# Duy1230/Map-Reduced-Approach-for-Vietnamese-Long-Document-Summarization

Hardware: AMD Instinct MI355X
Metric: map-phase chunks/sec (2k-tok chunk, 256-tok summary) at 1/2/4/8 MI355X (higher is better)
Workload: dtype f16

## Files before the change

### include/mapsum.h

```cpp
#ifndef MAPSUM_H
#define MAPSUM_H

#include <stddef.h>
#include <stdint.h>

#ifdef __cplusplus
extern "C" {
#endif

#define MS_ABI_VERSION 3

#define MS_OK 0
#define MS_EIO -5
#define MS_ENOMEM -12
#define MS_EBUSY -16
#define MS_EINVAL -22
#define MS_ENOSPC -28

#define MS_FINISH_EOS 1
#define MS_FINISH_LENGTH 2
#define MS_FINISH_ERROR 3

#define MS_FLAG_IGNORE_EOS 1u

// ... 71 lines not shown
int ms_quant_manifest(const ms_engine* e, int32_t* triples, int32_t cap);
int ms_declare_weight_q(ms_engine* e, int32_t tensor, int32_t layer, int32_t ggml_type);

int ms_submit(ms_engine* e, const int32_t* ids, int32_t n, int32_t num_predict,
              uint32_t flags, uint64_t tag);
int ms_set_eos_ids(ms_engine* e, const int32_t* ids, int32_t n);
int ms_step(ms_engine* e);
int ms_poll(ms_engine* e, ms_result* out, int32_t cap);
int ms_pending(const ms_engine* e);
int ms_get_stats(const ms_engine* e, ms_stats* out);
int ms_reset_stats(ms_engine* e);
int ms_set_profiling(ms_engine* e, uint32_t class_mask);
int ms_trace_push(const char* name);
int ms_trace_pop(void);
int ms_synchronize(ms_engine* e);
int ms_set_persist(ms_engine* e, int32_t on);
#define MS_DBG_KPOOL 0
#define MS_DBG_VPOOL 1
#define MS_DBG_DECODE_LOGITS 2
#define MS_DBG_DECODE_X 3
int ms_debug_read(ms_engine* e, int32_t which, int64_t offset, void* host, int64_t bytes);
int ms_debug_pk_stamps(uint64_t* out, int32_t n);
int ms_debug_a2_stamps(uint64_t* out, int32_t n);

int ms_forward(ms_engine* e, const int32_t* ids, int32_t n, int32_t n_layers_run,
               float* hidden_out, float* logits_out);
int ms_forward_packed(ms_engine* e, const int32_t* ids, const int32_t* lens, int32_t n_seqs,
                      int32_t n_layers_run, float* hidden_out, float* logits_out);
int ms_submit_forced(ms_engine* e, const int32_t* ids, int32_t n, const int32_t* forced,
                     int32_t n_forced, int32_t num_predict, uint32_t flags, uint64_t tag);

#define MS_EPI_STORE_F16 0
#define MS_EPI_ADD_F32 1
#define MS_EPI_SWIGLU 2
#define MS_EPI_STORE_F32 3
#define MS_EPI_ARGMAX 5
int ms_op_gemm(const void* A, const void* W, void* out, int32_t M, int32_t N, int32_t K,
               int32_t ldo, int32_t epilogue, void* stream);
int ms_op_gemm_resid(const void* A, const void* W, float* x, void* xg_out, const void* gamma, float* ssq_out,
                     int32_t M, int32_t N, int32_t K, void* stream);
int ms_gemm_resid_tiles(int32_t M, int32_t N);
int ms_set_gemm_variant(int32_t variant);
int ms_set_qgemv_gs(int32_t on);
int ms_set_attn_tuning(int32_t combine_grp, int32_t order);
int ms_set_dgemm_kh(int32_t kh);
int ms_set_dgemm_wn(int32_t wn);
// ... 35 lines not shown
```

### map-reduced-approach-for-vietnamese-long-document-summarization_amd/csrc/engine.cpp

```cpp
#include <hip/hip_runtime.h>

#include <algorithm>
#include <cmath>
#include <cstdio>
#include <cstdlib>
#include <cstring>
#include <deque>
#include <array>
#include <functional>
#include <map>
#include <tuple>
#include <memory>
#include <stdexcept>
#include <string>
#include <vector>

#if MS_HAVE_ROCTX
#include <rocprofiler-sdk-roctx/roctx.h>
#else
static inline int roctxRangePushA(const char*) { return 0; }
static inline int roctxRangePop() { return 0; }
#endif

#include "kernels.h"
// ... 128 lines not shown
  bool resid_fused(const QSlot* q) const {
    if (!resid_fuse || large_engine) return false;
    if (has_quant && !qresid_ok) return false;
    return !(q && q->ready()) || qresid;
  }
  int qlarge_min = 65;
  int qdgemm_mode = 1;
  int lm_gemm_min = 96;
  int qdf_min = 192;
  bool qdf(int M, int N, int K, int S, int epi) const {
    return !has_quant && qdf_min > 0 && cfg.max_batch >= qdf_min && qdgemm_f16_supported(M, N, K, S, epi);
  }
  bool large(int) const { return large_engine && (!has_quant || cfg.max_batch >= qlarge_min); }
  bool qd(const QSlot* q, int M, int N, int K, int S, int epi) const {
    if (!qdgemm_mode || !q || !q->ready()) return false;
    const QMat& m = q->m;
    const bool q4 = m.type0 == MS_QT_Q4_K && (m.n < 2 || m.type1 == MS_QT_Q4_K) && (m.n < 3 || m.type2 == MS_QT_Q4_K);
    return (q4 || qdgemm_mode == 2) && qdgemm_supported(M, N, K, S, epi, m);
  }
  bool row_groups(int B) const { return !large(B) && B > kMaxGemvRows; }
  int qsplit = 4;
  bool attn_slabs = true;
  RowScale cur_rs{};
  int32_t* args_d = nullptr;
  int32_t* args_h = nullptr;
  size_t args_cap = 0;
  struct Ctx {
    hipStream_t stream = nullptr;
    float* x = nullptr;
    float* ssq = nullptr;
    f16_t *xb = nullptr, *qkv = nullptr, *attn = nullptr, *hbuf = nullptr;
    float* logits = nullptr;
    int32_t* ids_out_d = nullptr;
    int32_t* args_d = nullptr;
    int32_t* args_h = nullptr;
    size_t args_cap = 0;
    hipEvent_t ev_a = nullptr, ev_b = nullptr;
  } cp, cd;
  bool overlap = false;
  void use(const Ctx& c) {
    stream = c.stream; x = c.x; ssq = c.ssq; xb = c.xb; qkv = c.qkv; attn = c.attn; hbuf = c.hbuf;
    logits = c.logits; ids_out_d = c.ids_out_d; args_d = c.args_d; args_h = c.args_h;
    args_cap = c.args_cap; ev_a = c.ev_a; ev_b = c.ev_b;
  }
  std::vector<uint8_t> stop_set;
  std::deque<std::unique_ptr<Seq>> waiting;
// ... 268 lines not shown
      attn_decode(DecodeQKV{qkv, nullptr, 0, cos_tab, sin_tab, RowScale{}}, kv, da);
    } else {
      prof_begin(K_ATTN_PREFILL);
      launch_attn_prefill(qkv, attn, Hq, Hk, kv, pa, stream);
      prof_end(K_ATTN_PREFILL);
    }
    const f16_t* g_next = l + 1 < L ? layers[l + 1].attn_norm : final_norm;
    if (decode) {
      gemm_or_gemv(attn, Ly.wo, x, T, H, Hq * D, H, MS_EPI_ADD_F32, decode, kc);
      norm_input(Ly.ffn_norm, T);
    } else {
      prefill_resid(attn, Ly.wo, T, Hq * D, Ly.ffn_norm);
    }
    const RowScale rs_ffn = cur_rs;
    gemm_or_gemv(xb, Ly.wgu, hbuf, T, 2 * F, H, F, MS_EPI_SWIGLU, decode, kc, &rs_ffn);
    if (decode) {
      gemm_or_gemv(hbuf, Ly.wdown, x, T, H, F, H, MS_EPI_ADD_F32, decode, kc);
      if (tail) norm_input(g_next, T);
    } else if (tail) {
      prefill_resid(hbuf, Ly.wdown, T, F, g_next);
    } else {
      gemm_or_gemv(hbuf, Ly.wdown, x, T, H, F, H, MS_EPI_ADD_F32, decode, kc);
    }
  }

  bool prefill_resid_ok(int T) const {
    const int tiles = gemm_resid_tiles(T, H);
    return tiles <= kGemmRsTiles && gemm_rs_tiles_ok(T, QKVN, tiles) && gemm_rs_tiles_ok(T, 2 * F, tiles);
  }
  void prefill_resid(const f16_t* X, const f16_t* W, int T, int K, const f16_t* g_next) {
    if (!prefill_resid_ok(T)) {
      gemm_or_gemv(X, W, x, T, H, K, H, MS_EPI_ADD_F32, false, K_GEMM);
      norm_input(g_next, T);
      return;
    }
    GemmResid gr{g_next, xb, ssq};
    prof_begin(K_GEMM);
    launch_gemm(X, W, x, T, H, K, H, MS_EPI_ADD_F32, stream, nullptr, &gr);
    prof_end(K_GEMM);
    cur_rs = make_row_scale(ssq, gemm_resid_tiles(T, H), H, cfg.norm_eps);
  }

  void norm_input(const f16_t* w, int T, const int32_t* row_idx = nullptr) {
    prof_begin(K_MISC);
    launch_rmsnorm(x, w, xb, ssq, T, H, row_idx, stream);
    prof_end(K_MISC);
// ... 210 lines not shown
    if (const char* v = getenv("MS_ATTN_SLABS")) E.attn_slabs = atoi(v) != 0;
    if (const char* v = getenv("MS_SPLIT_O")) E.split_o = atoi(v);
    if (const char* v = getenv("MS_SPLIT_DOWN")) E.split_down = atoi(v);
    if (const char* v = getenv("MS_DGEMM_MIN")) E.dgemm_min = atoi(v);
    E.large_engine = cfg->max_batch >= E.dgemm_min;
    if (const char* v = getenv("MS_QLARGE_MIN")) E.qlarge_min = atoi(v);
    if (const char* v = getenv("MS_QDGEMM")) E.qdgemm_mode = atoi(v);
    if (const char* v = getenv("MS_LM_GEMM_MIN")) E.lm_gemm_min = atoi(v);
    E.dgemm_kh = cfg->max_batch <= 128 && E.H % 128 == 0 ? dgemm_kh_setting() : 1;
    if (const char* v = getenv("MS_QDF_MIN")) E.qdf_min = atoi(v);
    if (E.qdf_min > 0 && cfg->max_batch >= E.qdf_min) {
      E.dsplit_qkv = 3;
      E.dsplit_down = 4;
    }
    if (const char* v = getenv("MS_DSPLIT_QKV")) E.dsplit_qkv = atoi(v);
    if (const char* v = getenv("MS_DSPLIT_O")) E.dsplit_o = atoi(v);
    if (const char* v = getenv("MS_DSPLIT_DOWN")) E.dsplit_down = atoi(v);
    if (const char* v = getenv("MS_DWN")) E.dwn_qkv = E.dwn_o = E.dwn_down = E.dwn_lm = atoi(v) == 8 ? 8 : 4;
    for (int* d : {&E.dsplit_qkv, &E.dsplit_o, &E.dsplit_down}) *d = std::min(std::max(*d, 1), (int)ms_engine::kMaxSplit);
    E.attn_ppw = attn_decode_ppw(cfg->max_batch, E.Hk, cfg->max_ctx);
    if (const char* v = getenv("MS_QSPLIT")) E.qsplit = atoi(v);
    if (const char* v = getenv("MS_RESID_FUSED")) E.resid_fuse = atoi(v) != 0;
    if (const char* v = getenv("MS_DECODE_TAIL")) E.tail_fuse = atoi(v) != 0;
    if (const char* v = getenv("MS_QRESID")) E.qresid = atoi(v) != 0;
    if (E.H % E.resid_rt || E.H / E.resid_rt > 256) E.resid_rt = 16;
    if (E.H % E.resid_rt || E.H / E.resid_rt > 256) E.resid_fuse = false;
    if (!gemv_rs_supported(cfg->max_batch, E.H / E.resid_rt)) E.resid_fuse = false;
    {
      const int Bg = std::min(cfg->max_batch, (int)ms_engine::kMaxGemvRows);
      E.qresid_ok = qgemv_supported(Bg, E.H, E.Hq * E.D, MS_GEMV_EPI_RESID_SSQ) &&
                    qgemv_supported(Bg, E.H, E.F, MS_GEMV_EPI_RESID_SSQ) &&
                    qgemv_supported(Bg, 2 * E.F, E.H, MS_GEMV_EPI_SWIGLU, E.H / E.resid_rt);
    }
    if (const char* v = getenv("MS_GRAPH_STEPS")) E.graph_steps = std::max(1, std::min(atoi(v), 16));
    for (ms_engine::Ctx* c : {&E.cp, &E.cd}) {
      c->args_cap = 8 * T + 64 * (size_t)cfg->max_batch + (size_t)cfg->max_batch * E.max_pages + 1024;
      c->args_d = E.dalloc<int32_t>(c->args_cap);
      HIP_OK(hipHostMalloc((void**)&c->args_h, c->args_cap * sizeof(int32_t), hipHostMallocDefault));
    }
    if (const char* v = getenv("MS_OVERLAP")) E.overlap = atoi(v) != 0;
    E.use(E.cp);
    HIP_OK(hipHostMalloc((void**)&E.ids_host, (size_t)ms_engine::kMaxRun * 256 * sizeof(int32_t),
                         hipHostMallocDefault));
    E.ids_ring_d = E.dalloc<int32_t>((size_t)ms_engine::kMaxRun * 256);
    {
      int dev_cu = 0;
// ... 451 lines not shown
    int q = 0;
    for (Seq* s : batch) { a.push_back(q); q += (int)s->prompt.size(); }
  }
  const size_t o_qlen = a.size();
  for (Seq* s : batch) a.push_back((int)s->prompt.size());
  const size_t o_kvlen = a.size();
  for (Seq* s : batch) a.push_back(s->len + (int)s->prompt.size());
  const size_t o_sslot = a.size();
  for (Seq* s : batch) a.push_back(s->slot);
  const size_t o_last = a.size();
  {
    int q = 0;
    for (Seq* s : batch) { q += (int)s->prompt.size(); a.push_back(q - 1); }
  }
  std::vector<std::pair<int, int32_t>> qb;
  for (int i = 0; i < S; ++i) {
    const int n = (int)batch[i]->prompt.size();
    for (int b = 0; b < (n + kPrefillQRows - 1) / kPrefillQRows; ++b)
      qb.push_back({batch[i]->len + b * kPrefillQRows, (i << 16) | b});
  }
  std::stable_sort(qb.begin(), qb.end(), [](auto& x, auto& y) { return x.first > y.first; });
  const size_t o_qblk = a.size();
  for (auto& p : qb) a.push_back(p.second);
  int32_t* d = E.upload_args(a);

  PrefillAttnArgs pa;
  pa.seq_qstart = d + o_qstart;
  pa.seq_qlen = d + o_qlen;
  pa.seq_kvlen = d + o_kvlen;
  pa.seq_slot = d + o_sslot;
  pa.qblk = d + o_qblk;
  pa.n_qblk = (int)qb.size();
  pa.cos_tab = E.cos_tab;
  pa.sin_tab = E.sin_tab;
  DecodeAttnArgs da{};

  E.prof_begin(K_MISC);
  launch_embed(d + o_ids, T, E.embed, E.H, E.x, E.stream);
  E.prof_end(K_MISC);
  E.norm_input(E.layers[0].attn_norm, T);
  for (int l = 0; l < n_layers_run; ++l)
    E.run_layer(l, T, false, d + o_pos, d + o_slot, pa, da, l + 1 < E.L || logits_all);
  HIP_OK(hipGetLastError());
  if (n_layers_run < E.L) return;
  if (!logits_all && !first_ids) return;
  if (logits_all) {
    launch_gemm(E.xb, E.lm_head, logits_all, T, E.V, E.H, E.V, MS_EPI_STORE_F32, E.stream, &E.cur_rs);
    return;
  }
  E.norm_input(E.final_norm, S, d + o_last);
  for (int r0 = 0; r0 < S; r0 += ms_engine::kMaxGemvRows) {
    const int rows = std::min(S - r0, (int)ms_engine::kMaxGemvRows);
    const RowScale rs = make_row_scale(E.ssq + r0, 1, E.H, E.cfg.norm_eps);
    E.gemm_or_gemv(E.xb + (size_t)r0 * E.H, E.lm_head, E.logits + (size_t)r0 * E.V, rows, E.V, E.H, E.V,
                   MS_EPI_STORE_F32, true, K_LMHEAD, &rs);
  }
  E.prof_begin(K_MISC);
  launch_argmax(E.logits, S, E.V, E.ids_out_d, E.stream);
  E.prof_end(K_MISC);
  HIP_OK(hipGetLastError());
  first_ids->resize(S);
  HIP_OK(hipMemcpyAsync(E.first_host, E.ids_out_d, S * sizeof(int32_t), hipMemcpyDeviceToHost, E.stream));
}

static void decode_head(ms_engine& E, int B, int32_t* d) {
  E.prof_begin(K_MISC);
  launch_embed(d, B, E.embed, E.H, E.x, E.stream, E.layers[0].attn_norm, E.xb, E.ssq);
  E.prof_end(K_MISC);
}

static void decode_tail(ms_engine& E, int B, int32_t* d, int tiles) {
  E.prof_begin(K_MISC);
  if (E.tail_fuse && B <= 256) {
// ... 354 lines not shown
      case MS_DBG_DECODE_X: base = E.cd.x; cap = (size_t)E.cfg.max_batch * E.H * sizeof(float); break;
      default: REQUIRE(false, MS_EINVAL, "ms_debug_read: unknown buffer");
    }
    REQUIRE((size_t)offset + (size_t)bytes <= cap, MS_EINVAL, "ms_debug_read: range past the buffer");
    HIP_OK(hipStreamSynchronize(E.cd.stream));
    HIP_OK(hipStreamSynchronize(E.cp.stream));
    HIP_OK(hipMemcpy(host, (const char*)base + offset, (size_t)bytes, hipMemcpyDeviceToHost));
    return MS_OK;
  });
}

int ms_debug_pk_stamps(uint64_t* out, int32_t n) {
  if (!out || n < 0) return MS_EINVAL;
  ms::persist_stamps(reinterpret_cast<unsigned long long*>(out), n);
  return MS_OK;
}

int ms_debug_a2_stamps(uint64_t* out, int32_t n) {
  if (!out || n < 0) return MS_EINVAL;
  ms::attn2_stamps(reinterpret_cast<unsigned long long*>(out), n);
  return MS_OK;
}

int ms_synchronize(ms_engine* e) {
  if (!e) return MS_EINVAL;
  return guarded(e, [&]() -> int {
    HIP_OK(hipStreamSynchronize(e->cp.stream));
    HIP_OK(hipStreamSynchronize(e->cd.stream));
    return MS_OK;
  });
}

int ms_forward_packed(ms_engine* e, const int32_t* ids, const int32_t* lens, int32_t n_seqs,
                      int32_t n_layers_run, float* hidden_out, float* logits_out) {
  if (!e) return MS_EINVAL;
  return guarded(e, [&]() -> int {
    ms_engine& E = *e;
    HIP_OK(hipSetDevice(E.cfg.device));
    REQUIRE(E.waiting.empty() && E.running.empty(), MS_EBUSY, "ms_forward needs an idle engine");
    REQUIRE(ids && lens && n_seqs >= 1 && n_seqs <= (int)E.free_slots.size(), MS_EINVAL,
            "bad probe batch (1 <= n_seqs <= max_batch)");
    REQUIRE(n_layers_run >= 0 && n_layers_run <= E.L, MS_EINVAL, "n_layers_run out of range");
    REQUIRE(!logits_out || n_layers_run == E.L, MS_EINVAL, "logits need every layer");
    int64_t T = 0, pages = 0;
    for (int i = 0; i < n_seqs; ++i) {
      REQUIRE(lens[i] >= 1 && lens[i] <= E.cfg.max_ctx, MS_EINVAL, "bad probe length");
// ... 332 lines not shown
```

### map-reduced-approach-for-vietnamese-long-document-summarization_amd/csrc/k_attn.hip

```cpp
#include <algorithm>

#include "attn_common.h"

namespace ms {

template <int GB>
__global__ __launch_bounds__(512, 1) void attn_prefill_kernel(const f16_t* __restrict__ qkv,
                                                              f16_t* __restrict__ out, int Hq,
                                                              int Hk, KVView kv, PrefillAttnArgs a,
                                                              float scale_log2) {
  constexpr int QR = kPrefillQRows;
  __shared__ __attribute__((aligned(16))) char smem[2 * 32768 + GB * QR * 256];
  const int tid = threadIdx.x, lane = tid & 63, wave = tid >> 6;
  const int g = lane >> 4, r = lane & 15;
  const int ngrp = Hq / GB;
  const int e = a.qblk[blockIdx.x / ngrp];
  const int h0 = (blockIdx.x % ngrp) * GB;
  const int sq = e >> 16, qb = e & 0xFFFF;
  const int qlen = a.seq_qlen[sq], kvlen = a.seq_kvlen[sq], qstart = a.seq_qstart[sq];
  const int slot = a.seq_slot[sq];
  const int kvh = h0 / (Hq / Hk);
  const int row_stride = (Hq + 2 * Hk) * kHeadDim;
  const int q0 = qb * QR + wave * 16;
  const int qi = q0 + r;
// ... 608 lines not shown
}
bool attn_decode2_supported(int B, int Hq, int Hk, int max_len, int ppb) {
  (void)B;
  if (Hk < 1 || Hq % Hk || Hq / Hk > kMaxGroup || ppb < kPpbMin || ppb > kPpbMax) return false;
  const int np = (max_len + kPage - 1) / kPage;
  return (np + ppb - 1) / ppb <= kMaxSplits && attn2_lds_bytes(ppb, Hq / Hk) <= 160 * 1024;
}

size_t attn_decode2_workspace_bytes(int B, int Hq, int max_len, int ppb) {
  const int np = (max_len + kPage - 1) / kPage;
  return (size_t)B * Hq * ((np + ppb - 1) / ppb) * 132 * sizeof(float);
}

constexpr int kA2StampBlocks = 1024, kA2Stamps = 32;
__device__ unsigned long long g_a2_stamps[kA2StampBlocks * kA2Stamps];
#define A2_STAMP(k)                                                                               \
  do {                                                                                            \
    if (stamps && lane == 0 && blockIdx.x < kA2StampBlocks)                                       \
      stamps[blockIdx.x * kA2Stamps + (k)] = __builtin_amdgcn_s_memrealtime();                    \
  } while (0)

template <bool FROM_SLABS, int PPB, bool TICKET>
__global__ __launch_bounds__(64 * PPB) void attn_decode2_kernel(
    DecodeQKV qa, int Hq, int Hk, KVView kv, DecodeAttnArgs a, float* __restrict__ ws, f16_t* __restrict__ out,
    int nsplit, float scale_log2, unsigned* __restrict__ cnt, unsigned long long* __restrict__ stamps) {
  extern __shared__ __attribute__((aligned(16))) char smem[];
  constexpr int NTHR = 64 * PPB;
  const int tid = threadIdx.x, lane = tid & 63;
  const int wave = __builtin_amdgcn_readfirstlane(tid >> 6);
  const int g = lane >> 4, r = lane & 15;
  const int BH = a.B * Hk;
  const int split = blockIdx.x / BH, grp = blockIdx.x - split * BH;
  const int b = grp / Hk, kvh = grp - b * Hk;
  const int G = Hq / Hk;
  const int len = a.seq_len[b];
  const int slot = a.seq_slot[b];
  const int np = (len + kPage - 1) / kPage;
  const int pg = split * PPB + wave;
  const int pos = len - 1;
  const int row_stride = (Hq + 2 * Hk) * kHeadDim;
  char* vs_ = smem + wave * 16384;
  float* raw = (float*)(smem + (size_t)PPB * 16384);
  f16_t* qn = (f16_t*)(raw + (G + 2) * kHeadDim);
  f16_t* kn = qn + G * kHeadDim;
  f16_t* vn = kn + kHeadDim;
  const bool has_page = pg < np;
  if (wave == PPB - 1) A2_STAMP(24);
  if (stamps && wave == 0) {
// ... 244 lines not shown
      out[(size_t)b * Hq * kHeadDim + (kvh * G + c) * kHeadDim + d] = f2h(O / L);
    }
    if (tid == 0) __hip_atomic_store(cnt + grp, 0u, __ATOMIC_RELAXED, __HIP_MEMORY_SCOPE_AGENT);
  }
}

void launch_attn_decode2(const DecodeQKV& qa, f16_t* out, int Hq, int Hk, KVView kv, DecodeAttnArgs a,
                         float* ws, int ppb, hipStream_t s, unsigned* cnt) {
  if (a.B <= 0) return;
  if (!attn_decode2_supported(a.B, Hq, Hk, a.max_len, ppb) || !kv.slot_major) return;
  if (qa.slabs && (qa.S < 1 || qa.S > kMaxSlabs)) return;
  if (qa.slabs && qa.rs.ssq && (qa.rs.tiles < 1 || qa.rs.tiles > 256)) return;
  const int np = (a.max_len + kPage - 1) / kPage;
  const int nsplit = (np + ppb - 1) / ppb;
  const float scale_log2 = kLog2e / sqrtf((float)kHeadDim);
  const dim3 grid(a.B * Hk * nsplit);
  const size_t lds = attn2_lds_bytes(ppb, Hq / Hk);
  static unsigned long long* stamps = [] {
    const char* e = getenv("MS_A2_STAMPS");
    void* p = nullptr;
    if (e && atoi(e)) (void)hipGetSymbolAddress(&p, HIP_SYMBOL(g_a2_stamps));
    return (unsigned long long*)p;
  }();
#define A2(P_)                                                                                                \
  case P_:                                                                                                    \
    if (qa.slabs && cnt)                                                                                      \
      MS_LAUNCH((attn_decode2_kernel<true, P_, true>), grid, dim3(64 * P_), lds, s, qa, Hq, Hk, kv, a, ws,    \
                out, nsplit, scale_log2, cnt, stamps);                                                        \
    else if (qa.slabs)                                                                                        \
      MS_LAUNCH((attn_decode2_kernel<true, P_, false>), grid, dim3(64 * P_), lds, s, qa, Hq, Hk, kv, a, ws,   \
                out, nsplit, scale_log2, cnt, stamps);                                                        \
    else                                                                                                      \
      MS_LAUNCH((attn_decode2_kernel<false, P_, false>), grid, dim3(64 * P_), lds, s, qa, Hq, Hk, kv, a, ws,  \
                out, nsplit, scale_log2, cnt, stamps);                                                        \
    break;
  switch (ppb) {
    A2(4) A2(5) A2(6) A2(7) A2(8) A2(9)
    default: return;
  }
#undef A2
  if (nsplit > 1 && !(qa.slabs && cnt)) launch_combine(ws, out, a.B, Hq, Hk, nsplit, combine_grp_ok(a.B, Hk), s);
}

}

namespace ms {
void attn2_stamps(unsigned long long* host, int n) {
  n = std::min(n, kA2StampBlocks * kA2Stamps);
  (void)hipMemcpyFromSymbol(host, HIP_SYMBOL(g_a2_stamps), (size_t)n * sizeof(unsigned long long));
}

void launch_attn_combine(const float* ws, f16_t* out, int B, int Hq, int Hk, int nsplit, hipStream_t s) {
  if (B <= 0 || nsplit <= 1) return;
  launch_combine(ws, out, B, Hq, Hk, nsplit, combine_grp_ok(B, Hk), s);
}
}
```

### map-reduced-approach-for-vietnamese-long-document-summarization_amd/csrc/k_gemv.hip

```cpp
#include "gemv_common.h"

namespace ms {

struct GemvPlan {
  int MT, NT, waves, U, tiles;
};

static GemvPlan gemv_plan(int M, int N, int K, int epi, int force_waves = 0, int rt = 0) {
  GemvPlan p;
  p.MT = (M + 15) / 16;
  p.NT = (epi == MS_GEMV_EPI_SWIGLU) ? 2 : 1;
  const int rows = p.NT == 1 && rt > 0 ? rt : 16 * p.NT;
  p.tiles = (N + rows - 1) / rows;
  const int steps = K / 64;
  int best_w = 0;
  if (force_waves > 0 && steps % force_waves == 0 && steps / force_waves <= 8) {
    best_w = force_waves;
  } else {
    for (int w = 16; w >= 1; --w)
      if (steps % w == 0 && steps / w <= 8) { best_w = w; break; }
  }
  p.waves = best_w;
  p.U = best_w ? steps / best_w : 0;
  return p;
}

size_t gemv_workspace_bytes(int, int, int) { return 256; }

constexpr size_t kMaxLds = 160 * 1024;

static size_t gemv_lds_main(const GemvPlan& p, int M, int K, bool xlds) {
  size_t xs = xlds ? gemv_x_lds_bytes(M, K) : 0;
  const size_t red = (size_t)p.waves * p.MT * p.NT * 256 * 4;
  return xs > red ? xs : red;
}
static size_t gemv_lds_bytes(const GemvPlan& p, int M, int K, bool xlds, const RowScale& rs = RowScale{}) {
  return gemv_lds_total(gemv_lds_main(p, M, K, xlds), rs, M);
}

template <int MT, int NT, int EPI, int U, int XM, bool RS>
__global__ __launch_bounds__(1024) void gemv_kernel(const f16_t* __restrict__ X,
                                                    const f16_t* __restrict__ W,
                                                    void* __restrict__ out, int M, int N, int K,
                                                    int ldk, int ldo, int rinv_off, GemvArgs ga) {
  extern __shared__ __attribute__((aligned(16))) char smem[];
  const int tid = threadIdx.x, lane = tid & 63, wave = tid >> 6;
  const int fr = lane & 15, fg = lane >> 4;
  const int rt = NT == 1 && ga.rt > 0 ? ga.rt : 16;
  const int n0 = blockIdx.x * (NT == 1 ? rt : 16 * NT);
  const int kbeg = wave * U * 64;
  if constexpr (EPI == MS_GEMV_EPI_STORE_F32) {
    X += (size_t)blockIdx.y * K;
    W += (size_t)blockIdx.y * K;
    out = (float*)out + (size_t)blockIdx.y * (ga.slab_rows > 0 ? ga.slab_rows : M) * ldo;
  }

  constexpr bool kRsEarly = XM == kXLds && NT == 1;
  if constexpr (RS) rs_begin<false>(smem, rinv_off, ga.rs, M);
  const ResidPre pre = resid_prefetch<EPI>(M, N, ldo, out, n0, ga);
  if constexpr (XM == kXLds) gemv_dma_x(smem, X, M, K, ldk);
  uint4 xr[XM == kXRegs ? U : 1][XM == kXRegs ? MT : 1][2];
  if constexpr (XM == kXRegs) {
#pragma unroll
    for (int u = 0; u < U; ++u)
#pragma unroll
      for (int m = 0; m < MT; ++m) {
        const f16_t* xg = X + (size_t)min(m * 16 + fr, M - 1) * ldk + kbeg + u * 64 + 16 * fg;
        xr[u][m][0] = ldg16(xg);
        xr[u][m][1] = ldg16(xg + 8);
      }
  }
  __builtin_amdgcn_sched_barrier(0);
  uint4 w[U][NT][2];
#pragma unroll
  for (int n = 0; n < NT; ++n) {
    const int wrow = NT == 1 ? n0 + min(fr, rt - 1) : n0 + n * 16 + fr;
    const f16_t* wp = W + (size_t)min(wrow, N - 1) * ldk + kbeg + 16 * fg;
#pragma unroll
    for (int u = 0; u < U; ++u) {
      w[u][n][0] = ldw16(wp + u * 64);
      w[u][n][1] = ldw16(wp + u * 64 + 8);
    }
  }
  if constexpr (XM == kXLds) {
    __builtin_amdgcn_sched_barrier(0);
    __builtin_amdgcn_s_waitcnt(vmcnt_imm(U * NT * 2));
    __builtin_amdgcn_s_barrier();
    if constexpr (RS && NT == 1) rs_finish<false>(smem, rinv_off, ga.rs, M, 0.f);
  }

  f32x4 acc[MT][NT];
#pragma unroll
  for (int m = 0; m < MT; ++m)
#pragma unroll
    for (int n = 0; n < NT; ++n) acc[m][n] = f32x4{0.f, 0.f, 0.f, 0.f};
#pragma unroll
  for (int u = 0; u < U; ++u) {
#pragma unroll
    for (int m = 0; m < MT; ++m) {
      const int xrow = min(m * 16 + fr, M - 1);
      f16x8 x0, x1;
      if constexpr (XM == kXRegs) {
        x0 = as_f16x8(xr[u][m][0]);
        x1 = as_f16x8(xr[u][m][1]);
      } else if constexpr (XM == kXLds) {
        const int k0 = kbeg + u * 64 + 16 * fg;
        x0 = *(const f16x8*)(smem + x_lds(xrow, k0, K));
        x1 = *(const f16x8*)(smem + x_lds(xrow, k0 + 8, K));
      } else {
        const f16_t* xg = X + (size_t)xrow * ldk + kbeg + u * 64 + 16 * fg;
        x0 = as_f16x8(ldg16(xg));
        x1 = as_f16x8(ldg16(xg + 8));
      }
#pragma unroll
      for (int n = 0; n < NT; ++n) {
        acc[m][n] = mfma16(x0, as_f16x8(w[u][n][0]), acc[m][n]);
        acc[m][n] = mfma16(x1, as_f16x8(w[u][n][1]), acc[m][n]);
      }
    }
  }
  gemv_finish<MT, NT, EPI, RS, kRsEarly, false>(acc, smem, rinv_off, M, N, ldo, out, n0, ga, pre);
}

template <int MT, int NT, int EPI, int U, bool RS>
static void gemv_go_rs(const f16_t* X, const f16_t* W, void* out, int M, int N, int K, int ldk,
                       const dim3& grid, const dim3& blk, size_t lds, int ro, int ldo, int xm,
                       const GemvArgs& ga, hipStream_t s) {
  if constexpr (MT * U <= kXRegsMaxFrags) {
    if (xm == kXRegs) {
      MS_LAUNCH((gemv_kernel<MT, NT, EPI, U, kXRegs, RS>), grid, blk, lds, s, X, W, out, M, N, K, ldk,
                ldo, ro, ga);
      return;
    }
  }
  if (xm == kXLds)
    MS_LAUNCH((gemv_kernel<MT, NT, EPI, U, kXLds, RS>), grid, blk, lds, s, X, W, out, M, N, K, ldk,
              ldo, ro, ga);
  else
    MS_LAUNCH((gemv_kernel<MT, NT, EPI, U, kXGlobal, RS>), grid, blk, lds, s, X, W, out, M, N, K, ldk,
              ldo, ro, ga);
}

template <int MT, int NT, int EPI, int U>
static void gemv_go(const f16_t* X, const f16_t* W, void* out, int M, int N, int K, int ldk,
                    int S, int ldo, const GemvPlan& p, size_t lds, int xm, const GemvArgs& ga,
                    hipStream_t s) {
  const dim3 grid(p.tiles, S), blk(64 * p.waves);
  const int ro = (int)gemv_rinv_offset(gemv_lds_main(p, M, K, xm == kXLds));
  if constexpr (EPI == MS_GEMV_EPI_ROPE_KV && MT != 1) {
    return;
  } else if constexpr (gemv_rs_epi<EPI>()) {
    if (ga.rs.ssq) gemv_go_rs<MT, NT, EPI, U, true>(X, W, out, M, N, K, ldk, grid, blk, lds, ro, ldo, xm, ga, s);
    else gemv_go_rs<MT, NT, EPI, U, false>(X, W, out, M, N, K, ldk, grid, blk, lds, ro, ldo, xm, ga, s);
  } else {
    gemv_go_rs<MT, NT, EPI, U, false>(X, W, out, M, N, K, ldk, grid, blk, lds, ro, ldo, xm, ga, s);
  }
}

template <int MT, int NT, int EPI>
static void gemv_go_u(const f16_t* X, const f16_t* W, void* out, int M, int N, int K, int ldk,
                      int S, int ldo, const GemvPlan& p, size_t lds, int xm, const GemvArgs& ga,
                      hipStream_t s) {
#define GU(U_) gemv_go<MT, NT, EPI, U_>(X, W, out, M, N, K, ldk, S, ldo, p, lds, xm, ga, s)
// ... 133 lines not shown
```

### map-reduced-approach-for-vietnamese-long-document-summarization_amd/csrc/k_misc.hip

```cpp
#include "gemv_common.h"

namespace ms {

thread_local ProfEvents* g_prof = nullptr;

__global__ __launch_bounds__(256) void embed_kernel(const int32_t* __restrict__ ids,
                                                    const f16_t* __restrict__ emb, int H,
                                                    float* __restrict__ x, const f16_t* __restrict__ gamma,
                                                    f16_t* __restrict__ xg, float* __restrict__ ssq) {
  __shared__ float red[4];
  const int t = blockIdx.x;
  const f16_t* row = emb + (size_t)ids[t] * H;
  float* xo = x + (size_t)t * H;
  float ss = 0.f;
  for (int c = threadIdx.x; c < H / 8; c += blockDim.x) {
    uint4 v = *(const uint4*)(row + c * 8);
    const uint32_t w[4] = {v.x, v.y, v.z, v.w};
    float4 a, b;
    a.x = h_lo(w[0]); a.y = h_hi(w[0]);
    a.z = h_lo(w[1]); a.w = h_hi(w[1]);
    b.x = h_lo(w[2]); b.y = h_hi(w[2]);
    b.z = h_lo(w[3]); b.w = h_hi(w[3]);
    *(float4*)(xo + c * 8) = a;
    *(float4*)(xo + c * 8 + 4) = b;
// ... 405 lines not shown
}

static uint64_t host_splitmix64(uint64_t z) {
  z += 0x9E3779B97F4A7C15ull;
  z = (z ^ (z >> 30)) * 0xBF58476D1CE4E5B9ull;
  z = (z ^ (z >> 27)) * 0x94D049BB133111EBull;
  return z ^ (z >> 31);
}

void launch_synth_linear(f16_t* dst, int kind, int layer, int rows, int cols, uint64_t seed,
                         float std, int map_mul, int map_add, hipStream_t s) {
  const float scale = (float)((double)std * 1.7320508075688772 / 65536.0);
  MS_LAUNCH(synth_linear_kernel, dim3(2048), dim3(256), 0, s, dst, kind, layer, rows,
                     cols, host_splitmix64(seed), scale, map_mul, map_add);
}

void launch_synth_norm(f16_t* dst, int kind, int layer, int n, uint64_t seed, float jitter,
                       hipStream_t s) {
  const float scale = (float)((double)jitter / 131070.0);
  MS_LAUNCH(synth_norm_kernel, dim3(16), dim3(256), 0, s, dst, kind, layer, n,
                     host_splitmix64(seed), scale);
}

__global__ void scatter_rows_kernel(const f16_t* __restrict__ src, f16_t* __restrict__ dst,
                                    int rows, int cols, int map_mul, int map_add) {
  const int r = blockIdx.x;
  const size_t dr = map_row(r, map_mul, map_add);
  for (int c = threadIdx.x; c < cols; c += blockDim.x) dst[dr * cols + c] = src[(size_t)r * cols + c];
}

void launch_scatter_rows(const f16_t* src, f16_t* dst, int rows, int cols, int map_mul,
                         int map_add, hipStream_t s) {
  MS_LAUNCH(scatter_rows_kernel, dim3(rows), dim3(256), 0, s, src, dst, rows, cols,
                     map_mul, map_add);
}

}
```

### map-reduced-approach-for-vietnamese-long-document-summarization_amd/csrc/kernels.h

```cpp
#pragma once
#include "common.h"

namespace ms {

struct KVView {
  f16_t* k;
  f16_t* v;
  const int32_t* block_table;
  int32_t max_pages;
  int32_t n_kv_heads;
  int32_t slot_major;
};

constexpr int kPrefillQRows = 128;
struct PrefillAttnArgs {
  const int32_t* seq_qstart;
  const int32_t* seq_qlen;
  const int32_t* seq_kvlen;
  const int32_t* seq_slot;
  const int32_t* qblk;
  int32_t n_qblk;
  const float* cos_tab;
  const float* sin_tab;
};
// ... 9 lines not shown
struct RowScale {
  const float* ssq;
  int tiles, H;
  float eps;
  float inv_h;
};
inline RowScale make_row_scale(const float* ssq, int tiles, int H, float eps) {
  return RowScale{ssq, tiles, H, eps, 1.0f / (float)H};
}
constexpr float kXgScale = 0.0625f, kXgUnscale = 16.0f;
__device__ __forceinline__ float rs_rinv(float sum, const RowScale& rs) {
  return __builtin_amdgcn_rsqf(__fmaf_rn(sum, rs.inv_h, rs.eps)) * kXgUnscale;
}

void launch_embed(const int32_t* ids, int T, const f16_t* emb, int H, float* x, hipStream_t s,
                  const f16_t* gamma = nullptr, f16_t* xg = nullptr, float* ssq = nullptr);
void launch_decode_advance(int32_t* args, const int32_t* ids_out, int32_t* ring, int B, int V,
                           hipStream_t s);
void launch_decode_tail(const void* partials, int tiles, int32_t* args, int32_t* ids_out, int32_t* ring, int B,
                        int V, const f16_t* emb, int H, float* x, const f16_t* gamma, f16_t* xg, float* ssq,
                        hipStream_t s);
void launch_rmsnorm(const float* x, const f16_t* w, f16_t* y, float* ssq, int rows, int H,
                    const int32_t* row_idx, hipStream_t s);
void launch_rope_kv(f16_t* qkv, int T, int Hq, int Hk, const int32_t* tok_pos,
                    const int32_t* tok_slot, const float* cos_tab, const float* sin_tab,
                    KVView kv, hipStream_t s, bool rope_q = true);
void launch_argmax(const float* logits, int rows, int n, int32_t* out, hipStream_t s);

struct GemmResid {
  const f16_t* gamma;
  f16_t* xg;
  float* ssq;
};
constexpr int kGemmRsTiles = 24;
constexpr int kGemmStatCols = 128;
int gemm_resid_tiles(int M, int N);
bool gemm_rs_tiles_ok(int M, int N, int tiles);
void launch_gemm(const f16_t* A, const f16_t* W, void* out, int M, int N, int K, int ldo,
                 int epi, hipStream_t s, const RowScale* rs = nullptr, const GemmResid* gr = nullptr);
void set_gemm_variant(int v);
void set_qgemv_gs(bool on);
void set_attn_tuning(int combine_grp, int order);
void set_dgemm_kh(int kh);
void set_dgemm_wn(int wn);
enum {
  MS_GEMV_EPI_STORE_F16 = 0,
// ... 81 lines not shown
                         PrefillAttnArgs a, hipStream_t s);
struct DecodeQKV {
  const f16_t* qkv;
  const float* slabs;
  int S;
  const float* cos_tab;
  const float* sin_tab;
  RowScale rs;
};
size_t attn_decode_workspace_bytes(int B, int Hq, int max_len);
bool attn_decode_supported(int B, int Hq, int Hk, int max_len);
int attn_decode_ppw(int max_batch, int Hk, int max_ctx);
void launch_attn_decode(const DecodeQKV& qa, f16_t* out, int Hq, int Hk, KVView kv,
                        DecodeAttnArgs a, float* ws, hipStream_t s);
int attn_decode2_ppb(int max_batch, int Hk, int max_ctx);
bool attn_decode2_supported(int B, int Hq, int Hk, int max_len, int ppb);
size_t attn_decode2_workspace_bytes(int B, int Hq, int max_len, int ppb);
void launch_attn_decode2(const DecodeQKV& qa, f16_t* out, int Hq, int Hk, KVView kv, DecodeAttnArgs a,
                         float* ws, int ppb, hipStream_t s, unsigned* cnt = nullptr);

void launch_attn_combine(const float* ws, f16_t* out, int B, int Hq, int Hk, int nsplit, hipStream_t s);

void attn2_stamps(unsigned long long* host, int n);

struct PkLayer {
  const f16_t* wqkv;
  const f16_t* wo;
  const f16_t* wgu;
  const f16_t* wdown;
  const f16_t* ffn_norm;
  const f16_t* g_next;
  f16_t* kc;
  f16_t* vc;
  const char* packed;
};

struct PkArgs {
  PkLayer layers[28];
  int L, B;
  const int32_t* seq_len;
  const int32_t* seq_slot;
  int max_pages, ppb, nsplit_ws;
  const float* cos_tab;
  const float* sin_tab;
  float eps, inv_h, scale_log2;
  int rs0_tiles;
// ... 40 lines not shown
```

### map-reduced-approach-for-vietnamese-long-document-summarization_amd/mapsum/_lib.py

```python
from __future__ import annotations

import ctypes as C
import os

_HERE = os.path.dirname(os.path.abspath(__file__))
LIB_PATH = os.environ.get("MAPSUM_LIB") or os.path.join(_HERE, "libmapsum.so")

MS_ABI_VERSION = 3
MS_OK, MS_EIO, MS_ENOMEM, MS_EBUSY, MS_EINVAL, MS_ENOSPC = 0, -5, -12, -16, -22, -28
MS_FINISH_EOS, MS_FINISH_LENGTH, MS_FINISH_ERROR = 1, 2, 3
MS_FLAG_IGNORE_EOS = 1
(MS_T_EMBED, MS_T_ATTN_NORM, MS_T_WQ, MS_T_WK, MS_T_WV, MS_T_WO, MS_T_FFN_NORM, MS_T_WGATE,
 MS_T_WUP, MS_T_WDOWN, MS_T_FINAL_NORM, MS_T_LM_HEAD) = range(12)
MS_EPI_STORE_F16, MS_EPI_ADD_F32, MS_EPI_SWIGLU, MS_EPI_STORE_F32 = range(4)
MS_EPI_ARGMAX = 5
GEMM_DEFAULT = 4
MS_GGML_Q4_K, MS_GGML_Q6_K = 12, 14
K_GEMM, K_ATTN_PREFILL, K_GEMV, K_ATTN_DECODE, K_LMHEAD, K_MISC, K_PERSIST = range(7)
MS_DBG_KPOOL, MS_DBG_VPOOL, MS_DBG_DECODE_LOGITS, MS_DBG_DECODE_X = range(4)

EXPORTED = (
    "ms_create", "ms_destroy", "ms_last_error", "ms_load_weight", "ms_init_synthetic",
    "ms_load_weight_q", "ms_init_synthetic_q", "ms_op_dequant", "ms_op_quant_rows", "ms_op_qgemv", "ms_op_qgemv_split", "ms_op_qdgemm",
    "ms_submit", "ms_step", "ms_poll", "ms_pending", "ms_get_stats", "ms_reset_stats",
    "ms_set_profiling", "ms_synchronize", "ms_forward", "ms_op_gemm", "ms_op_gemv_workspace",
    "ms_op_gemv", "ms_op_gemv_tuned", "ms_op_gemv_split", "ms_op_dgemm", "ms_op_residual_rmsnorm", "ms_op_rmsnorm",
    "ms_op_argmax", "ms_op_argmax_partials", "ms_set_gemm_variant", "ms_set_qgemv_gs", "ms_set_attn_tuning", "ms_set_dgemm_kh", "ms_set_dgemm_wn",
    "ms_weight_regions", "ms_quant_manifest", "ms_declare_weight_q",
    "ms_forward_packed", "ms_submit_forced", "ms_set_eos_ids", "ms_op_gemv_strided",
    "ms_op_gemv_resid", "ms_op_set_row_scale", "ms_op_gemm_resid", "ms_gemm_resid_tiles",
    "ms_trace_push", "ms_trace_pop", "ms_debug_a2_stamps", "ms_set_persist", "ms_debug_read", "ms_debug_pk_stamps",
)


class MsConfig(C.Structure):
    _fields_ = [("abi_version", C.c_int32),
                ("n_layers", C.c_int32), ("hidden", C.c_int32), ("n_heads", C.c_int32),
                ("n_kv_heads", C.c_int32), ("head_dim", C.c_int32), ("ffn", C.c_int32),
                ("vocab", C.c_int32),
                ("rope_theta", C.c_float), ("rope_factor", C.c_float),
                ("rope_low_freq_factor", C.c_float), ("rope_high_freq_factor", C.c_float),
                ("rope_orig_ctx", C.c_int32), ("norm_eps", C.c_float), ("tie_embeddings", C.c_int32),
                ("device", C.c_int32), ("max_batch", C.c_int32), ("max_ctx", C.c_int32),
                ("max_prefill_tokens", C.c_int32), ("n_pages", C.c_int32), ("n_eos", C.c_int32),
                ("eos_ids", C.c_int32 * 8)]


class MsResult(C.Structure):
    _fields_ = [("tag", C.c_uint64), ("ids", C.POINTER(C.c_int32)), ("n_ids", C.c_int32),
                ("finish_reason", C.c_int32), ("n_prompt", C.c_int32), ("_pad", C.c_int32)]


class MsStats(C.Structure):
    _fields_ = [("prefill_tokens", C.c_int64), ("decode_tokens", C.c_int64),
# ... 56 lines not shown
        "ms_op_gemv_workspace": (i64, [i32, i32, i32]),
        "ms_op_gemv": (i32, [vp, vp, vp, i32, i32, i32, i32, i32, vp, vp]),
        "ms_op_gemv_tuned": (i32, [vp, vp, vp, i32, i32, i32, i32, i32, vp, i32, vp]),
        "ms_op_gemv_split": (i32, [vp, vp, vp, i32, i32, i32, i32, i32, vp]),
        "ms_op_dgemm": (i32, [vp, vp, vp, i32, i32, i32, i32, i32, i32, vp]),
        "ms_op_residual_rmsnorm": (i32, [vp, vp, i32, vp, vp, vp, i32, i32, vp]),
        "ms_op_rmsnorm": (i32, [vp, vp, vp, vp, i32, i32, vp, vp]),
        "ms_set_gemm_variant": (i32, [i32]),
        "ms_set_qgemv_gs": (i32, [i32]),
        "ms_set_attn_tuning": (i32, [i32, i32]),
        "ms_set_dgemm_kh": (i32, [i32]),
        "ms_set_dgemm_wn": (i32, [i32]),
        "ms_op_argmax": (i32, [vp, i32, i32, vp, vp]),
        "ms_op_argmax_partials": (i32, [vp, i32, i32, vp, vp]),
        "ms_weight_regions": (i32, [vp, C.POINTER(vp), C.POINTER(i64), i32]),
        "ms_quant_manifest": (i32, [vp, pi32, i32]),
        "ms_declare_weight_q": (i32, [vp, i32, i32, i32]),
        "ms_trace_push": (i32, [C.c_char_p]),
        "ms_trace_pop": (i32, []),
        "ms_set_persist": (i32, [vp, i32]),
        "ms_debug_read": (i32, [vp, i32, i64, vp, i64]),
        "ms_debug_pk_stamps": (i32, [vp, i32]),
        "ms_debug_a2_stamps": (i32, [vp, i32]),
    }
    for name, (res, args) in sig.items():
        if ab and not hasattr(lib, name):
            continue
        fn = getattr(lib, name)
        fn.restype = res
        fn.argtypes = args
    return lib


def check(rc: int, handle=None, what: str = "") -> int:
    if rc < 0:
        msg = load().ms_last_error(handle)
        raise RuntimeError(f"libmapsum {what} failed ({rc}): {msg.decode() if msg else ''}")
    return rc


class trace:

    def __init__(self, name: str):
        self.name = name.encode()
        self.lib = None

# ... 15 lines not shown
```

Measured before the change: 12.90.

## Trim last prefill layer to last-token rows and add gemv timing stamps

During prefill with first-token sampling only, the final layer now computes QKV and KV writes for all tokens, but runs attention only for the query blocks holding each sequence's last token. It then gathers those last rows and runs the O-projection, FFN and final norm on just S rows instead of T. This is meant to remove most of the last layer's post-attention GEMM work. The change also adds optional per-block realtime stamps to the gemv kernel and repacks the decode attention kernel's arguments, both of which add kernel parameters on the hot paths.

```diff
diff --git a/include/mapsum.h b/include/mapsum.h
--- a/include/mapsum.h
+++ b/include/mapsum.h
@@ -117,6 +117,7 @@
 int ms_debug_read(ms_engine* e, int32_t which, int64_t offset, void* host, int64_t bytes);
 int ms_debug_pk_stamps(uint64_t* out, int32_t n);
 int ms_debug_a2_stamps(uint64_t* out, int32_t n);
+int ms_debug_gemv_stamps(uint64_t* out, int32_t n);
 
 int ms_forward(ms_engine* e, const int32_t* ids, int32_t n, int32_t n_layers_run,
                float* hidden_out, float* logits_out);
diff --git a/map-reduced-approach-for-vietnamese-long-document-summarization_amd/csrc/engine.cpp b/map-reduced-approach-for-vietnamese-long-document-summarization_amd/csrc/engine.cpp
--- a/map-reduced-approach-for-vietnamese-long-document-summarization_amd/csrc/engine.cpp
+++ b/map-reduced-approach-for-vietnamese-long-document-summarization_amd/csrc/engine.cpp
@@ -174,6 +174,9 @@
   int qsplit = 4;
   bool attn_slabs = true;
   RowScale cur_rs{};
+  bool prefill_trim = true;
+  float* last_x = nullptr;
+  f16_t* last_attn = nullptr;
   int32_t* args_d = nullptr;
   int32_t* args_h = nullptr;
   size_t args_cap = 0;
@@ -488,6 +491,39 @@
     } else {
       gemm_or_gemv(hbuf, Ly.wdown, x, T, H, F, H, MS_EPI_ADD_F32, decode, kc);
     }
+  }
+
+  void run_last_layer_trimmed(int l, int T, int S, const int32_t* tok_pos, const int32_t* tok_slot,
+                              const PrefillAttnArgs& pa_last, const int32_t* last_row) {
+    const Layer& Ly = layers[l];
+    const RowScale rs_attn = cur_rs;
+    KVView kv = kv_layer(l);
+    gemm_or_gemv(xb, Ly.wqkv, qkv, T, QKVN, H, QKVN, MS_EPI_STORE_F16, false, K_GEMM, &rs_attn);
+    prof_begin(K_MISC);
+    launch_rope_kv(qkv, T, Hq, Hk, tok_pos, tok_slot, cos_tab, sin_tab, kv, stream, !pa_last.cos_tab);
+    prof_end(K_MISC);
+    prof_begin(K_ATTN_PREFILL);
+    launch_attn_prefill(qkv, attn, Hq, Hk, kv, pa_last, stream);
+    prof_end(K_ATTN_PREFILL);
+    prof_begin(K_MISC);
+    launch_gather_rows(x, last_x, H, attn, last_attn, Hq * D, last_row, S, stream);
+    prof_end(K_MISC);
+    if (prefill_resid_ok(S)) {
+      GemmResid gr{Ly.ffn_norm, xb, ssq};
+      prof_begin(K_GEMM);
+      launch_gemm(last_attn, Ly.wo, last_x, S, H, Hq * D, H, MS_EPI_ADD_F32, stream, nullptr, &gr);
+      prof_end(K_GEMM);
+      cur_rs = make_row_scale(ssq, gemm_resid_tiles(S, H), H, cfg.norm_eps);
+    } else {
+      gemm_or_gemv(last_attn, Ly.wo, last_x, S, H, Hq * D, H, MS_EPI_ADD_F32, false, K_GEMM);
+      prof_begin(K_MISC);
+      launch_rmsnorm(last_x, Ly.ffn_norm, xb, ssq, S, H, nullptr, stream);
+      prof_end(K_MISC);
+      cur_rs = norm_rs();
+    }
+    const RowScale rs_ffn = cur_rs;
+    gemm_or_gemv(xb, Ly.wgu, hbuf, S, 2 * F, H, F, MS_EPI_SWIGLU, false, K_GEMM, &rs_ffn);
+    gemm_or_gemv(hbuf, Ly.wdown, last_x, S, H, F, H, MS_EPI_ADD_F32, false, K_GEMM);
   }
 
   bool prefill_resid_ok(int T) const {
@@ -744,6 +780,9 @@
     if (const char* v = getenv("MS_QSPLIT")) E.qsplit = atoi(v);
     if (const char* v = getenv("MS_RESID_FUSED")) E.resid_fuse = atoi(v) != 0;
     if (const char* v = getenv("MS_DECODE_TAIL")) E.tail_fuse = atoi(v) != 0;
+    if (const char* v = getenv("MS_PREFILL_TRIM")) E.prefill_trim = atoi(v) != 0;
+    E.last_x = E.dalloc<float>((size_t)cfg->max_batch * E.H);
+    E.last_attn = E.dalloc<f16_t>((size_t)cfg->max_batch * E.Hq * E.D);
     if (const char* v = getenv("MS_QRESID")) E.qresid = atoi(v) != 0;
     if (E.H % E.resid_rt || E.H / E.resid_rt > 256) E.resid_rt = 16;
     if (E.H % E.resid_rt || E.H / E.resid_rt > 256) E.resid_fuse = false;
@@ -1241,6 +1280,12 @@
   std::stable_sort(qb.begin(), qb.end(), [](auto& x, auto& y) { return x.first > y.first; });
   const size_t o_qblk = a.size();
   for (auto& p : qb) a.push_back(p.second);
+  const bool trim = E.prefill_trim && first_ids && !logits_all && n_layers_run == E.L;
+  const size_t o_qblk_last = a.size();
+  if (trim)
+    for (auto& p : qb)
+      if ((p.second & 0xFFFF) == ((int)batch[p.second >> 16]->prompt.size() - 1) / kPrefillQRows)
+        a.push_back(p.second);
   int32_t* d = E.upload_args(a);
 
   PrefillAttnArgs pa;
@@ -1258,8 +1303,14 @@
   launch_embed(d + o_ids, T, E.embed, E.H, E.x, E.stream);
   E.prof_end(K_MISC);
   E.norm_input(E.layers[0].attn_norm, T);
-  for (int l = 0; l < n_layers_run; ++l)
+  for (int l = 0; l < n_layers_run - (trim ? 1 : 0); ++l)
     E.run_layer(l, T, false, d + o_pos, d + o_slot, pa, da, l + 1 < E.L || logits_all);
+  if (trim) {
+    PrefillAttnArgs pl = pa;
+    pl.qblk = d + o_qblk_last;
+    pl.n_qblk = S;
+    E.run_last_layer_trimmed(E.L - 1, T, S, d + o_pos, d + o_slot, pl, d + o_last);
+  }
   HIP_OK(hipGetLastError());
   if (n_layers_run < E.L) return;
   if (!logits_all && !first_ids) return;
@@ -1267,7 +1318,13 @@
     launch_gemm(E.xb, E.lm_head, logits_all, T, E.V, E.H, E.V, MS_EPI_STORE_F32, E.stream, &E.cur_rs);
     return;
   }
-  E.norm_input(E.final_norm, S, d + o_last);
+  if (trim) {
+    E.prof_begin(K_MISC);
+    launch_rmsnorm(E.last_x, E.final_norm, E.xb, E.ssq, S, E.H, nullptr, E.stream);
+    E.prof_end(K_MISC);
+  } else {
+    E.norm_input(E.final_norm, S, d + o_last);
+  }
   for (int r0 = 0; r0 < S; r0 += ms_engine::kMaxGemvRows) {
     const int rows = std::min(S - r0, (int)ms_engine::kMaxGemvRows);
     const RowScale rs = make_row_scale(E.ssq + r0, 1, E.H, E.cfg.norm_eps);
@@ -1668,6 +1725,12 @@
   return MS_OK;
 }
 
+int ms_debug_gemv_stamps(uint64_t* out, int32_t n) {
+  if (!out || n < 0) return MS_EINVAL;
+  ms::gemv_stamps(reinterpret_cast<unsigned long long*>(out), n);
+  return MS_OK;
+}
+
 int ms_synchronize(ms_engine* e) {
   if (!e) return MS_EINVAL;
   return guarded(e, [&]() -> int {
diff --git a/map-reduced-approach-for-vietnamese-long-document-summarization_amd/csrc/k_attn.hip b/map-reduced-approach-for-vietnamese-long-document-summarization_amd/csrc/k_attn.hip
--- a/map-reduced-approach-for-vietnamese-long-document-summarization_amd/csrc/k_attn.hip
+++ b/map-reduced-approach-for-vietnamese-long-document-summarization_amd/csrc/k_attn.hip
@@ -654,8 +654,21 @@
 
 template <bool FROM_SLABS, int PPB, bool TICKET>
 __global__ __launch_bounds__(64 * PPB) void attn_decode2_kernel(
-    DecodeQKV qa, int Hq, int Hk, KVView kv, DecodeAttnArgs a, float* __restrict__ ws, f16_t* __restrict__ out,
-    int nsplit, float scale_log2, unsigned* __restrict__ cnt, unsigned long long* __restrict__ stamps) {
+    f16_t* kpool, f16_t* vpool, int max_pages, int n_kv_heads, const int32_t* __restrict__ seq_len,
+    const int32_t* __restrict__ seq_slot, int B, int Hk, int Hq, int nsplit, const float* __restrict__ slabs,
+    DecodeQKV qa_, KVView kv_, DecodeAttnArgs a_, float* __restrict__ ws, f16_t* __restrict__ out,
+    float scale_log2, unsigned* __restrict__ cnt, unsigned long long* __restrict__ stamps) {
+  DecodeQKV qa = qa_;
+  qa.slabs = slabs;
+  KVView kv = kv_;
+  kv.k = kpool;
+  kv.v = vpool;
+  kv.max_pages = max_pages;
+  kv.n_kv_heads = n_kv_heads;
+  DecodeAttnArgs a = a_;
+  a.seq_len = seq_len;
+  a.seq_slot = seq_slot;
+  a.B = B;
   extern __shared__ __attribute__((aligned(16))) char smem[];
   constexpr int NTHR = 64 * PPB;
   const int tid = threadIdx.x, lane = tid & 63;
@@ -946,23 +959,26 @@
     if (e && atoi(e)) (void)hipGetSymbolAddress(&p, HIP_SYMBOL(g_a2_stamps));
     return (unsigned long long*)p;
   }();
+#define A2_LEAD                                                                                               \
+  kv.k, kv.v, kv.max_pages, kv.n_kv_heads, a.seq_len, a.seq_slot, a.B, Hk, Hq, nsplit, qa.slabs
 #define A2(P_)                                                                                                \
   case P_:                                                                                                    \
     if (qa.slabs && cnt)                                                                                      \
-      MS_LAUNCH((attn_decode2_kernel<true, P_, true>), grid, dim3(64 * P_), lds, s, qa, Hq, Hk, kv, a, ws,    \
-                out, nsplit, scale_log2, cnt, stamps);                                                        \
+      MS_LAUNCH((attn_decode2_kernel<true, P_, true>), grid, dim3(64 * P_), lds, s, A2_LEAD, qa, kv, a, ws,   \
+                out, scale_log2, cnt, stamps);                                                                \
     else if (qa.slabs)                                                                                        \
-      MS_LAUNCH((attn_decode2_kernel<true, P_, false>), grid, dim3(64 * P_), lds, s, qa, Hq, Hk, kv, a, ws,   \
-                out, nsplit, scale_log2, cnt, stamps);                                                        \
+      MS_LAUNCH((attn_decode2_kernel<true, P_, false>), grid, dim3(64 * P_), lds, s, A2_LEAD, qa, kv, a, ws,  \
+                out, scale_log2, cnt, stamps);                                                                \
     else                                                                                                      \
-      MS_LAUNCH((attn_decode2_kernel<false, P_, false>), grid, dim3(64 * P_), lds, s, qa, Hq, Hk, kv, a, ws,  \
-                out, nsplit, scale_log2, cnt, stamps);                                                        \
+      MS_LAUNCH((attn_decode2_kernel<false, P_, false>), grid, dim3(64 * P_), lds, s, A2_LEAD, qa, kv, a, ws, \
+                out, scale_log2, cnt, stamps);                                                                \
     break;
   switch (ppb) {
     A2(4) A2(5) A2(6) A2(7) A2(8) A2(9)
     default: return;
   }
 #undef A2
+#undef A2_LEAD
   if (nsplit > 1 && !(qa.slabs && cnt)) launch_combine(ws, out, a.B, Hq, Hk, nsplit, combine_grp_ok(a.B, Hk), s);
 }
 
diff --git a/map-reduced-approach-for-vietnamese-long-document-summarization_amd/csrc/k_gemv.hip b/map-reduced-approach-for-vietnamese-long-document-summarization_amd/csrc/k_gemv.hip
--- a/map-reduced-approach-for-vietnamese-long-document-summarization_amd/csrc/k_gemv.hip
+++ b/map-reduced-approach-for-vietnamese-long-document-summarization_amd/csrc/k_gemv.hip
@@ -1,4 +1,8 @@
 #include "gemv_common.h"
+
+#include <algorithm>
+#include <tuple>
+#include <vector>
 
 namespace ms {
 
@@ -38,17 +42,23 @@
   return gemv_lds_total(gemv_lds_main(p, M, K, xlds), rs, M);
 }
 
+constexpr int kGemvStampSlots = 8, kGemvStampBlocks = 2048, kGemvStamps = 8;
+__device__ unsigned long long g_gemv_stamps[kGemvStampSlots * kGemvStampBlocks * kGemvStamps];
+
 template <int MT, int NT, int EPI, int U, int XM, bool RS>
 __global__ __launch_bounds__(1024) void gemv_kernel(const f16_t* __restrict__ X,
                                                     const f16_t* __restrict__ W,
                                                     void* __restrict__ out, int M, int N, int K,
-                                                    int ldk, int ldo, int rinv_off, GemvArgs ga) {
+                                                    int ldk, int ldo, int rinv_off, int rt_arg,
+                                                    GemvArgs ga, unsigned long long* __restrict__ stamps) {
   extern __shared__ __attribute__((aligned(16))) char smem[];
   const int tid = threadIdx.x, lane = tid & 63, wave = tid >> 6;
   const int fr = lane & 15, fg = lane >> 4;
-  const int rt = NT == 1 && ga.rt > 0 ? ga.rt : 16;
+  const int rt = NT == 1 && rt_arg > 0 ? rt_arg : 16;
   const int n0 = blockIdx.x * (NT == 1 ? rt : 16 * NT);
   const int kbeg = wave * U * 64;
+  unsigned long long ts[5] = {0, 0, 0, 0, 0};
+  if (stamps) ts[0] = __builtin_amdgcn_s_memrealtime();
   if constexpr (EPI == MS_GEMV_EPI_STORE_F32) {
     X += (size_t)blockIdx.y * K;
     W += (size_t)blockIdx.y * K;
@@ -71,6 +81,7 @@
       }
   }
   __builtin_amdgcn_sched_barrier(0);
+  if (stamps) ts[1] = __builtin_amdgcn_s_memrealtime();
   uint4 w[U][NT][2];
 #pragma unroll
   for (int n = 0; n < NT; ++n) {
@@ -82,6 +93,7 @@
       w[u][n][1] = ldw16(wp + u * 64 + 8);
     }
   }
+  if (stamps) ts[2] = __builtin_amdgcn_s_memrealtime();
   if constexpr (XM == kXLds) {
     __builtin_amdgcn_sched_barrier(0);
     __builtin_amdgcn_s_waitcnt(vmcnt_imm(U * NT * 2));
@@ -89,6 +101,10 @@
     if constexpr (RS && NT == 1) rs_finish<false>(smem, rinv_off, ga.rs, M, 0.f);
   }
 
+  if (stamps) {
+    __builtin_amdgcn_s_waitcnt(vmcnt_imm(0));
+    ts[3] = __builtin_amdgcn_s_memrealtime();
+  }
   f32x4 acc[MT][NT];
 #pragma unroll
   for (int m = 0; m < MT; ++m)
@@ -119,26 +135,63 @@
       }
     }
   }
+  if (stamps) ts[4] = __builtin_amdgcn_s_memrealtime();
   gemv_finish<MT, NT, EPI, RS, kRsEarly, false>(acc, smem, rinv_off, M, N, ldo, out, n0, ga, pre);
+  if (stamps && tid == 0) {
+    const unsigned blk = blockIdx.y * gridDim.x + blockIdx.x;
+    if (blk < (unsigned)kGemvStampBlocks) {
+      unsigned long long* p = stamps + (size_t)blk * kGemvStamps;
+#pragma unroll
+      for (int i = 0; i < 5; ++i) p[i] = ts[i];
+      p[5] = __builtin_amdgcn_s_memrealtime();
+      p[6] = ((unsigned long long)(unsigned)N << 32) | (unsigned)K;
+      p[7] = ((unsigned long long)(unsigned)EPI << 32) | (gridDim.x * gridDim.y);
+    }
+  }
+}
+
+static std::vector<std::tuple<int, int, int>> g_gemv_stamp_keys;
+static unsigned long long* gemv_stamp_slot(int N, int K, int epi) {
+  static unsigned long long* base = [] {
+    const char* e = getenv("MS_GEMV_STAMPS");
+    void* p = nullptr;
+    if (e && atoi(e)) (void)hipGetSymbolAddress(&p, HIP_SYMBOL(g_gemv_stamps));
+    return (unsigned long long*)p;
+  }();
+  if (!base) return nullptr;
+  const auto key = std::make_tuple(N, K, epi);
+  size_t i = 0;
+  while (i < g_gemv_stamp_keys.size() && g_gemv_stamp_keys[i] != key) ++i;
+  if (i == g_gemv_stamp_keys.size()) {
+    if (i >= (size_t)kGemvStampSlots) return nullptr;
+    g_gemv_stamp_keys.push_back(key);
+  }
+  return base + i * (size_t)kGemvStampBlocks * kGemvStamps;
+}
+
+void gemv_stamps(unsigned long long* host, int n) {
+  n = std::min(n, kGemvStampSlots * kGemvStampBlocks * kGemvStamps);
+  (void)hipMemcpyFromSymbol(host, HIP_SYMBOL(g_gemv_stamps), (size_t)n * sizeof(unsigned long long));
 }
 
 template <int MT, int NT, int EPI, int U, bool RS>
 static void gemv_go_rs(const f16_t* X, const f16_t* W, void* out, int M, int N, int K, int ldk,
                        const dim3& grid, const dim3& blk, size_t lds, int ro, int ldo, int xm,
                        const GemvArgs& ga, hipStream_t s) {
+  unsigned long long* st = gemv_stamp_slot(N, K, EPI);
   if constexpr (MT * U <= kXRegsMaxFrags) {
     if (xm == kXRegs) {
       MS_LAUNCH((gemv_kernel<MT, NT, EPI, U, kXRegs, RS>), grid, blk, lds, s, X, W, out, M, N, K, ldk,
-                ldo, ro, ga);
+                ldo, ro, ga.rt, ga, st);
       return;
     }
   }
   if (xm == kXLds)
     MS_LAUNCH((gemv_kernel<MT, NT, EPI, U, kXLds, RS>), grid, blk, lds, s, X, W, out, M, N, K, ldk,
-              ldo, ro, ga);
+              ldo, ro, ga.rt, ga, st);
   else
     MS_LAUNCH((gemv_kernel<MT, NT, EPI, U, kXGlobal, RS>), grid, blk, lds, s, X, W, out, M, N, K, ldk,
-              ldo, ro, ga);
+              ldo, ro, ga.rt, ga, st);
 }
 
 template <int MT, int NT, int EPI, int U>
diff --git a/map-reduced-approach-for-vietnamese-long-document-summarization_amd/csrc/k_misc.hip b/map-reduced-approach-for-vietnamese-long-document-summarization_amd/csrc/k_misc.hip
--- a/map-reduced-approach-for-vietnamese-long-document-summarization_amd/csrc/k_misc.hip
+++ b/map-reduced-approach-for-vietnamese-long-document-summarization_amd/csrc/k_misc.hip
@@ -451,6 +451,26 @@
                      host_splitmix64(seed), scale);
 }
 
+__global__ __launch_bounds__(256) void gather_rows_kernel(const float* __restrict__ x, float* __restrict__ xc,
+                                                          int H, const f16_t* __restrict__ at,
+                                                          f16_t* __restrict__ atc, int A,
+                                                          const int32_t* __restrict__ row_idx) {
+  const int r = blockIdx.x;
+  const size_t src = (size_t)row_idx[r];
+  const uint4* xs = (const uint4*)(x + src * H);
+  uint4* xd = (uint4*)(xc + (size_t)r * H);
+  for (int c = threadIdx.x; c < H / 4; c += 256) xd[c] = xs[c];
+  const uint4* as = (const uint4*)(at + src * A);
+  uint4* ad = (uint4*)(atc + (size_t)r * A);
+  for (int c = threadIdx.x; c < A / 8; c += 256) ad[c] = as[c];
+}
+
+void launch_gather_rows(const float* x, float* xc, int H, const f16_t* at, f16_t* atc, int A,
+                        const int32_t* row_idx, int rows, hipStream_t s) {
+  if (rows <= 0) return;
+  MS_LAUNCH(gather_rows_kernel, dim3(rows), dim3(256), 0, s, x, xc, H, at, atc, A, row_idx);
+}
+
 __global__ void scatter_rows_kernel(const f16_t* __restrict__ src, f16_t* __restrict__ dst,
                                     int rows, int cols, int map_mul, int map_add) {
   const int r = blockIdx.x;
diff --git a/map-reduced-approach-for-vietnamese-long-document-summarization_amd/csrc/kernels.h b/map-reduced-approach-for-vietnamese-long-document-summarization_amd/csrc/kernels.h
--- a/map-reduced-approach-for-vietnamese-long-document-summarization_amd/csrc/kernels.h
+++ b/map-reduced-approach-for-vietnamese-long-document-summarization_amd/csrc/kernels.h
@@ -55,6 +55,8 @@
                         hipStream_t s);
 void launch_rmsnorm(const float* x, const f16_t* w, f16_t* y, float* ssq, int rows, int H,
                     const int32_t* row_idx, hipStream_t s);
+void launch_gather_rows(const float* x, float* xc, int H, const f16_t* at, f16_t* atc, int A,
+                        const int32_t* row_idx, int rows, hipStream_t s);
 void launch_rope_kv(f16_t* qkv, int T, int Hq, int Hk, const int32_t* tok_pos,
                     const int32_t* tok_slot, const float* cos_tab, const float* sin_tab,
                     KVView kv, hipStream_t s, bool rope_q = true);
@@ -182,6 +184,7 @@
 void launch_attn_combine(const float* ws, f16_t* out, int B, int Hq, int Hk, int nsplit, hipStream_t s);
 
 void attn2_stamps(unsigned long long* host, int n);
+void gemv_stamps(unsigned long long* host, int n);
 
 struct PkLayer {
   const f16_t* wqkv;
diff --git a/map-reduced-approach-for-vietnamese-long-document-summarization_amd/mapsum/_lib.py b/map-reduced-approach-for-vietnamese-long-document-summarization_amd/mapsum/_lib.py
--- a/map-reduced-approach-for-vietnamese-long-document-summarization_amd/mapsum/_lib.py
+++ b/map-reduced-approach-for-vietnamese-long-document-summarization_amd/mapsum/_lib.py
@@ -29,7 +29,7 @@
     "ms_weight_regions", "ms_quant_manifest", "ms_declare_weight_q",
     "ms_forward_packed", "ms_submit_forced", "ms_set_eos_ids", "ms_op_gemv_strided",
     "ms_op_gemv_resid", "ms_op_set_row_scale", "ms_op_gemm_resid", "ms_gemm_resid_tiles",
-    "ms_trace_push", "ms_trace_pop", "ms_debug_a2_stamps", "ms_set_persist", "ms_debug_read", "ms_debug_pk_stamps",
+    "ms_trace_push", "ms_trace_pop", "ms_debug_a2_stamps", "ms_debug_gemv_stamps", "ms_set_persist", "ms_debug_read", "ms_debug_pk_stamps",
 )
 
 
@@ -132,6 +132,7 @@
         "ms_debug_read": (i32, [vp, i32, i64, vp, i64]),
         "ms_debug_pk_stamps": (i32, [vp, i32]),
         "ms_debug_a2_stamps": (i32, [vp, i32]),
+        "ms_debug_gemv_stamps": (i32, [vp, i32]),
     }
     for name, (res, args) in sig.items():
         if ab and not hasattr(lib, name):
```

Result: no change. 13.02 (median of 6 runs) (+1.0%).
